# jperezrua/mfas

Hardware: AMD Instinct MI355X
Metric: candidate-archs trained/sec (NTU inner loop) (higher is better)
Workload: dtype f32

## Files before the change

include/mfas_hip.h:

```cpp
#ifndef MFAS_HIP_H
#define MFAS_HIP_H

#include <stdint.h>

#ifdef __cplusplus
extern "C" {
#endif

#define MFAS_OK 0
#define MFAS_EINVAL -1
#define MFAS_EHIP -2
#define MFAS_ENOMEM -3

#define MFAS_MAX_CELLS 4
#define MFAS_MAX_TAPS 8

#define MFAS_DT_F32 0
#define MFAS_DT_BF16 1
#define MFAS_DT_F16 2

typedef struct mfas_hyper {
    int32_t R;
    int32_t C;
    int32_t B;
// ... 74 lines not shown
int mfas_population_forward(mfas_population* pop, int32_t k, const mfas_table* tab, int64_t row0,
                            int64_t nrows, float* logits, int64_t* corrects);

int mfas_population_forward_train(mfas_population* pop, int32_t k, const mfas_table* tab, int64_t row0, int32_t nrows,
                                  int32_t step_index, float* logits);

int mfas_population_backward(mfas_population* pop, int32_t k, const mfas_table* table, int64_t row0, int32_t nrows,
                             int32_t step_index, const float* dlogits);

int mfas_population_sweep_profile(const mfas_population* pop, int64_t* launches, double* total_ms,
                                  double* bytes_per_launch);
int mfas_population_set_profiling(mfas_population* pop, int32_t on);

int mfas_population_schedule(const mfas_population* pop, int32_t info[8]);

int mfas_population_plan(const mfas_hyper* hp, const int32_t* confs, const int32_t* n_cells, int32_t K, int32_t device,
                         int32_t chunk_cols, int32_t info[8]);

int mfas_stream_probe(int64_t bytes_per_plane, int32_t iters, double* gb_per_s);

int mfas_global_pool(const void* x, int32_t dtype, int64_t rows, int64_t inner, void* out, int32_t out_dtype,
                     void* hip_stream);

int mfas_range_push(const char* name);
int mfas_range_pop(void);

int mfas_tuning_describe(char* buf, int32_t cap);

int mfas_population_set_best_threshold(mfas_population* pop, double threshold);

// ... 7 lines not shown
```

mfas_amd/_lib.py:

```python
import ctypes as C
import os

_HERE = os.path.dirname(os.path.abspath(__file__))
LIB_PATH = os.environ.get("MFAS_LIB") or os.path.join(_HERE, "csrc", "libmfas_hip.so")

MFAS_DT = {"float32": 0, "bfloat16": 1, "float16": 2}
MAX_TAPS = 8


class mfas_hyper(C.Structure):
    _fields_ = [("R", C.c_int32), ("C", C.c_int32), ("B", C.c_int32), ("bn", C.c_int32),
                ("alphas", C.c_int32), ("multitask", C.c_int32), ("drpt", C.c_double),
                ("wd", C.c_double), ("beta1", C.c_double), ("beta2", C.c_double),
                ("adam_eps", C.c_double), ("bn_eps", C.c_double), ("bn_momentum", C.c_double),
                ("s_sizes", C.c_int32 * MAX_TAPS), ("v_sizes", C.c_int32 * MAX_TAPS), ("loss_mode", C.c_int32),
                ("allow_plain_cell", C.c_int32), ("f1_threshold", C.c_double), ("tap_bits", C.c_int32), ("order_per_candidate", C.c_int32)]


class mfas_table(C.Structure):
    _fields_ = [("s", C.c_void_p * MAX_TAPS), ("v", C.c_void_p * MAX_TAPS), ("vlogit", C.c_void_p),
                ("slogit", C.c_void_p), ("label", C.c_void_p), ("multilabel", C.c_void_p), ("N", C.c_int64),
                ("dtype", C.c_int32), ("_pad", C.c_int32)]


# ... 23 lines not shown
    L.mfas_population_destroy.argtypes = [P]
    L.mfas_population_destroy.restype = None
    L.mfas_population_param_count.argtypes = [P, C.c_int32]
    L.mfas_population_param_count.restype = C.c_int64
    L.mfas_population_set_params.argtypes = [P, C.c_int32, P]
    L.mfas_population_get_params.argtypes = [P, C.c_int32, C.c_int32, P]
    L.mfas_population_init.argtypes = [P, P]
    L.mfas_population_train.argtypes = [P, C.POINTER(mfas_table), C.POINTER(mfas_table), P, P, C.c_int32,
                                        C.c_int64, C.c_int32, P, P]
    L.mfas_population_forward.argtypes = [P, C.c_int32, C.POINTER(mfas_table), C.c_int64, C.c_int64, P, P]
    L.mfas_population_forward_train.argtypes = [P, C.c_int32, C.POINTER(mfas_table), C.c_int64, C.c_int32, C.c_int32, P]
    L.mfas_population_backward.argtypes = [P, C.c_int32, C.POINTER(mfas_table), C.c_int64, C.c_int32, C.c_int32, P]
    L.mfas_population_sweep_profile.argtypes = [P, P, P, P]
    L.mfas_population_schedule.argtypes = [P, P]
    L.mfas_population_plan.argtypes = [C.POINTER(mfas_hyper), P, P, C.c_int32, C.c_int32, C.c_int32, P]
    L.mfas_population_set_profiling.argtypes = [P, C.c_int32]
    L.mfas_population_set_pos_weight.argtypes = [P, P]
    L.mfas_stream_probe.argtypes = [C.c_int64, C.c_int32, P]
    L.mfas_global_pool.argtypes = [P, C.c_int32, C.c_int64, C.c_int64, P, C.c_int32, P]
    L.mfas_range_push.argtypes = [C.c_char_p]
    L.mfas_population_init_torch_streams.argtypes = [P, P, P, C.c_double, C.c_double]
    L.mfas_tuning_describe.argtypes = [C.c_char_p, C.c_int32]
    L.mfas_population_train_from.argtypes = [P, C.POINTER(mfas_table), C.POINTER(mfas_table), P, P, C.c_int32,
                                             C.c_int32, C.c_int32, C.c_int32, P, P]
    L.mfas_population_set_state.argtypes = [P, C.c_int32, C.c_int32, P]
    L.mfas_population_get_progress.argtypes = [P, C.c_int32, P, P, P, P]
    L.mfas_population_set_progress.argtypes = [P, C.c_int32, P, P, P, P]
    L.mfas_population_move.argtypes = [P, C.c_int32, P, C.c_int32]
    _lib = L
    return L


EXPORTS = ["mfas_last_error", "mfas_version", "mfas_population_create", "mfas_population_destroy",
           "mfas_population_param_count", "mfas_population_set_params", "mfas_population_get_params",
           "mfas_population_init", "mfas_population_train", "mfas_population_forward",
           "mfas_population_sweep_profile", "mfas_population_set_profiling", "mfas_population_set_pos_weight", "mfas_global_pool", "mfas_stream_probe", "mfas_source_digest",
           "mfas_population_set_best_threshold", "mfas_population_forward_train", "mfas_population_schedule",
           "mfas_population_plan", "mfas_population_backward", "mfas_range_push", "mfas_range_pop", "mfas_population_init_torch_streams", "mfas_tuning_describe",
           "mfas_population_train_from", "mfas_population_set_state", "mfas_population_get_progress", "mfas_population_set_progress",
           "mfas_population_move"]


def tuning() -> dict:
    buf = C.create_string_buffer(2048)
    check(lib().mfas_tuning_describe(buf, 2048))
    return dict(kv.split("=", 1) for kv in buf.value.decode().split())


import contextlib


@contextlib.contextmanager
def profiler_range(name: str):
    L = lib()
    L.mfas_range_push(name.encode())
# ... 10 lines not shown
```

mfas_amd/csrc/launches.hip.h:

```cpp
#pragma once
#include <stdint.h>
#include <vector>

struct Launch {
    int sweep_g = -1, upd = 0, fwd = 0;
    int64_t sweep_t = 0;
    int chain_g = -1;
    int64_t chain_t = 0;
    int gather_g = -1, gather_n = 0;
    int64_t gather_b = 0;
};

static void epoch_launches(int ngroups, bool same_group, int64_t T, bool gather, std::vector<Launch>& out) {
    out.clear();
    gather = gather && ngroups == 2;
    auto add = [&](int gs, int upd, int fwd, int64_t ts, int gc, int64_t tc) -> Launch& {
        out.push_back(Launch{gs, upd, fwd, ts, gc, tc});
        return out.back();
    };
    auto rows = [&](Launch& l, int g, int64_t b, int n) { if (gather) { l.gather_g = g; l.gather_b = b; l.gather_n = n; } };
    for (int g = 0; g < ngroups; ++g) rows(add(g, 0, 1, 0, -1, 0), g, 0, T > 1 ? 2 : 1);
    if (ngroups == 1 && same_group) {
        for (int64_t t = 0; t < T; ++t) add(0, 1, t + 1 < T, t, 0, t);
    } else if (ngroups == 1) {
        for (int64_t t = 0; t < T; ++t) { add(-1, 0, 0, 0, 0, t); add(0, 1, t + 1 < T, t, -1, 0); }
    } else {
        add(-1, 0, 0, 0, 0, 0);
        for (int64_t t = 0; t < T; ++t) {
            const int fwd = t + 1 < T;
            Launch& a = add(0, 1, fwd, t, 1, t);
            if (t >= 1 && t + 1 < T) rows(a, 1, t + 1, 1);
            Launch& b = add(1, 1, fwd, t, fwd ? 0 : -1, t + 1);
            if (fwd && t + 2 < T) rows(b, 0, t + 2, 1);
        }
    }
}
```

mfas_amd/csrc/mfas_hip.hip:

```cpp
#include <hip/hip_runtime.h>
#include <hip/hip_fp16.h>
#pragma clang fp contract(off)
#include <stdint.h>
#include <stdio.h>
#include <string.h>
#include <math.h>
#include <algorithm>
#include <string>
#include <vector>
#include <thread>
#include <chrono>
#include <dlfcn.h>

#include "mfas_hip.h"

#include "common.hip.h"
#include "sweep.hip.h"
#include "chain.hip.h"

struct StepArgs {
    SweepArgs sa;
    ChainArgs ca;
    int32_t nchain, _pad;
    GatherArgs ga;
// ... 36 lines not shown
}

#include "wide.hip.h"
#include "persist.hip.h"
#include "eval.hip.h"
#include "pack.hip.h"

#include "plan.hip.h"

struct mfas_population {
    mfas_hyper hp;
    Tuning tune;
    int K = 0, device = 0, n_cus = 0;
    int chunk_cols_req = 0;
    hipStream_t stream = nullptr;
    LayoutPlan plan;
    float* plane = nullptr;
    float* wt = nullptr;
    float* stepbuf = nullptr;
    float* best = nullptr;
    CandDev* d_cands = nullptr;
    SegDesc* d_descs = nullptr;
    struct GroupDev { SegDesc* d_descs = nullptr; TapDesc* d_taps = nullptr; };
    std::vector<GroupDev> groups;
    DevStats* d_stats = nullptr;
    int32_t* d_status = nullptr;
    uint32_t* d_seeds = nullptr;
    long long* d_corr = nullptr;
    float* d_posw = nullptr;
    int stats_cap = 0;
// ... 188 lines not shown
    CREATE_CHK(hipMalloc(&p->d_corr, sizeof(long long)));
    CREATE_CHK(upload(&p->d_posw, std::vector<float>(pl.g.Cp, 1.0f)));
    CREATE_CHK(upload(&p->d_cands, pl.cands));
    CREATE_CHK(upload(&p->d_descs, pl.descs));
    p->groups.resize(pl.groups.size());
    for (size_t gi = 0; gi < pl.groups.size(); ++gi) {
        CREATE_CHK(upload(&p->groups[gi].d_descs, pl.groups[gi].descs));
        CREATE_CHK(upload(&p->groups[gi].d_taps, pl.groups[gi].taps));
    }
    if (pl.red_in_sweep) {
        CREATE_CHK(hipMalloc(&p->d_red_cnt, sizeof(uint32_t) * K * MFAS_MAX_CELLS));
        CREATE_CHK(hipMemset(p->d_red_cnt, 0, sizeof(uint32_t) * K * MFAS_MAX_CELLS));
    }
    if (pl.same_group) CREATE_CHK(hipMalloc(&p->d_cellflag, sizeof(uint32_t) * K * CELLFLAG_STRIDE));
    if (pl.chain_split) CREATE_CHK(hipMalloc(&p->d_xch, sizeof(float) * (size_t)K * XCH_CAND_FLOATS));
    CREATE_CHK(hipMemsetAsync(p->plane, 0, sizeof(float) * 3 * (size_t)pl.plane_stride, p->stream));
    CREATE_CHK(hipMemsetAsync(p->wt, 0, sizeof(float) * wt_floats, p->stream));
    CREATE_CHK(hipMemsetAsync(p->stepbuf, 0, sizeof(float) * (size_t)pl.step_total, p->stream));
    CREATE_CHK(set_lds_all(pl));
    if (pl.persist) {
        CREATE_CHK(upload(&p->d_pdescs, pl.pdescs));
        CREATE_CHK(upload(&p->d_need, pl.need));
        CREATE_CHK(upload(&p->d_role, pl.role));
        CREATE_CHK(hipMalloc(&p->d_sync, sizeof(uint32_t) * ((size_t)K * PERSIST_SYNC_STRIDE + 64)));
        if (p->tune.persist_trace) {
            CREATE_CHK(hipMalloc(&p->d_trace, sizeof(unsigned long long) * 256));
            CREATE_CHK(hipMemset(p->d_trace, 0, sizeof(unsigned long long) * 256));
        }
    }
    CREATE_CHK(hipStreamSynchronize(p->stream));
// ... 12 lines not shown
                                    int32_t chunk_cols, int32_t info[8]) {
    if (!info) return fail(MFAS_EINVAL, "null argument or K <= 0");
    if (int vrc = validate_inputs(hp, confs, n_cells, K)) return vrc;
    const int ncu = device_cus(device);
    LayoutPlan pl;
    if (int prc = plan_layout(hp, confs, n_cells, nullptr, K, chunk_cols, ncu, true, tuning_from_env(), pl)) return prc;
    info[0] = pl.persist ? 1 : 0; info[1] = pl.nres; info[2] = pl.nres_wg; info[3] = pl.res_nu;
    info[4] = pl.chunk; info[5] = (pl.lean_chain ? 1 : 0) | (pl.wide ? 2 : 0); info[6] = ncu; info[7] = K;
    return MFAS_OK;
}

extern "C" void mfas_population_destroy(mfas_population* p) {
    if (!p) return;
    hipSetDevice(p->device);
    hipStreamSynchronize(p->stream);
    for (hipEvent_t e : p->ev) hipEventDestroy(e);
    hipFree(p->plane); hipFree(p->wt); hipFree(p->stepbuf); hipFree(p->best);
    for (auto& gr : p->groups) { hipFree(gr.d_descs); hipFree(gr.d_taps); }
    hipFree(p->d_cands); hipFree(p->d_descs); hipFree(p->d_stats); hipFree(p->d_status);
    hipFree(p->d_seeds); hipFree(p->d_corr); hipFree(p->d_posw);
    hipFree(p->d_red_cnt);
    hipFree(p->d_gather);
    hipFree(p->d_cellflag);
    hipFree(p->d_xch);
    hipFree(p->d_move);
    hipFree(p->d_sync); hipFree(p->d_need); hipFree(p->d_role); hipFree(p->d_scal); hipFree(p->d_trace); hipFree(p->d_pdescs);
    delete p;
}

extern "C" int64_t mfas_population_param_count(const mfas_population* p, int32_t k) {
// ... 214 lines not shown
}

extern "C" int mfas_population_set_best_threshold(mfas_population* p, double threshold) {
    if (!p) return fail(MFAS_EINVAL, "null");
    p->best_threshold = threshold;
    return MFAS_OK;
}

extern "C" int mfas_population_set_profiling(mfas_population* p, int32_t on) {
    if (!p) return fail(MFAS_EINVAL, "null");
    p->profiling = on != 0;
    p->prof_every = p->tune.prof_every;
    return MFAS_OK;
}

extern "C" int mfas_population_schedule(const mfas_population* p, int32_t info[8]) {
    if (!p || !info) return fail(MFAS_EINVAL, "null");
    const LayoutPlan& pl = p->plan;
    info[0] = pl.persist ? 1 : 0; info[1] = pl.nres; info[2] = pl.nres_wg; info[3] = pl.res_nu;
    info[4] = pl.res_chain ? 1 : 0; info[5] = (pl.lean_chain ? 1 : 0) | (pl.wide ? 2 : 0) | (std::max(1, pl.chain_split) << 8); info[6] = pl.same_group ? -1 : (int32_t)pl.groups.size(); info[7] = p->K;
    return MFAS_OK;
}

extern "C" int mfas_population_sweep_profile(const mfas_population* p, int64_t* launches, double* total_ms,
                                             double* bytes_per_launch) {
    if (!p) return fail(MFAS_EINVAL, "null");
    if (launches) *launches = p->prof_launches;
    if (total_ms) *total_ms = p->prof_ms;
    if (bytes_per_launch) *bytes_per_launch = p->bytes_per_launch;
    return MFAS_OK;
}
```

mfas_amd/csrc/plan.hip.h:

```cpp
#pragma once
struct Tuning {
    int persist = -1;
    int no_lean_chain = 0;
    int groups = 0;
    int same_group = -1;
    int no_tap_major = 0;
    int force_tap_major = 0;
    int no_red_in_sweep = 0;
    double occ_bytes = -1.0;
    int no_xcd_placement = 0;
    int n_xcd = 0;
    int persist_trace = 0;
    int nt = -1;
    int eval_no_x16 = 0;
    int eval_no_msplit = 0;
    int eval_no_b3 = 0;
    int eval_no_wl = 0;
    int no_gather = 0;
    int gather_verbose = 0;
    int no_plain_chain = 0;
    int persist_verbose = 0;
    int prof_every = 16;
    int chain_split = -1;
    int test_not_resident = -1;
    int test_lose_step = -1;
};

static Tuning tuning_from_env() {
    Tuning t;
    auto flag = [](const char* n) { return getenv(n) ? 1 : 0; };
    auto num = [](const char* n, int dflt) { const char* e = getenv(n); return e ? atoi(e) : dflt; };
    t.persist = getenv("MFAS_PERSIST") ? (atoi(getenv("MFAS_PERSIST")) != 0 ? 1 : 0) : -1;
    t.no_lean_chain = flag("MFAS_NO_LEAN_CHAIN");
    t.groups = num("MFAS_GROUPS", 0);
    t.same_group = num("MFAS_SAME_GROUP", -1);
    t.no_tap_major = flag("MFAS_NO_TAP_MAJOR");
    t.force_tap_major = flag("MFAS_FORCE_TAP_MAJOR");
    t.no_red_in_sweep = flag("MFAS_NO_RED_IN_SWEEP");
    if (const char* e = getenv("MFAS_OCC_BYTES")) t.occ_bytes = atof(e);
    t.no_xcd_placement = flag("MFAS_NO_XCD_PLACEMENT");
    t.n_xcd = num("MFAS_XCDS", 0);
    t.persist_trace = flag("MFAS_PERSIST_TRACE");
    t.nt = getenv("MFAS_NT") ? (atoi(getenv("MFAS_NT")) != 0 ? 1 : 0) : -1;
    t.eval_no_x16 = flag("MFAS_EVAL_NO_X16");
    t.eval_no_msplit = flag("MFAS_EVAL_NO_MSPLIT");
    t.eval_no_b3 = flag("MFAS_EVAL_NO_B3");
    t.eval_no_wl = flag("MFAS_EVAL_NO_WL");
    t.no_gather = flag("MFAS_NO_GATHER");
    t.gather_verbose = flag("MFAS_GATHER_VERBOSE");
    t.no_plain_chain = flag("MFAS_NO_PLAIN_CHAIN");
    t.persist_verbose = num("MFAS_PERSIST_VERBOSE", 0);
    t.prof_every = std::max(1, num("MFAS_PROF_EVERY", 16));
    t.chain_split = num("MFAS_CHAIN_SPLIT", -1);
#ifdef MFAS_TEST_HOOKS
    t.test_not_resident = num("MFAS_PERSIST_TEST_NOT_RESIDENT", -1);
    t.test_lose_step = num("MFAS_PERSIST_TEST_LOSE_STEP", -1);
#endif
    return t;
}

extern "C" int mfas_tuning_describe(char* buf, int32_t cap) {
    if (!buf || cap <= 0) return MFAS_EINVAL;
    const Tuning t = tuning_from_env();
    char tmp[1024];
    snprintf(tmp, sizeof(tmp),
             "persist=%d no_lean_chain=%d groups=%d same_group=%d "
             "no_tap_major=%d force_tap_major=%d no_red_in_sweep=%d occ_bytes=%g no_xcd_placement=%d n_xcd=%d persist_trace=%d nt=%d eval_no_x16=%d "
             "eval_no_msplit=%d eval_no_b3=%d eval_no_wl=%d no_gather=%d gather_verbose=%d no_plain_chain=%d persist_verbose=%d prof_every=%d "
             "chain_split=%d test_not_resident=%d test_lose_step=%d hooks=%d",
             t.persist, t.no_lean_chain, t.groups, t.same_group,
             t.no_tap_major, t.force_tap_major, t.no_red_in_sweep, t.occ_bytes, t.no_xcd_placement, t.n_xcd, t.persist_trace, t.nt, t.eval_no_x16,
             t.eval_no_msplit, t.eval_no_b3, t.eval_no_wl, t.no_gather, t.gather_verbose, t.no_plain_chain, t.persist_verbose, t.prof_every,
             t.chain_split, t.test_not_resident, t.test_lose_step,
#ifdef MFAS_TEST_HOOKS
             1
#else
             0
#endif
    );
    snprintf(buf, (size_t)cap, "%s", tmp);
    return MFAS_OK;
}

static inline int ceil16(int x) { return (x + 15) & ~15; }

static int pick_chunk(int cols_p, int target) {
    int best = 16;
    for (int c = 16; c <= cols_p && c <= target; c += 16)
        if (cols_p % c == 0) best = c;
    return best;
}

static int validate_inputs(const mfas_hyper* hp, const int32_t* confs, const int32_t* n_cells, int32_t K) {
    if (!hp || !confs || !n_cells || K <= 0) return fail(MFAS_EINVAL, "null argument or K <= 0");
// ... 156 lines not shown
    std::vector<int64_t> nparams;
    std::vector<int64_t> cand_plane_base, cand_plane_size;
    int64_t plane_stride = 0, wt_size = 0, step_total = 0;
    double bytes_per_launch = 0.0;
    bool persist = false;
    bool res_chain = false;
    bool res_wide = false;
    int nres = 0;
    int res_nu = 1;
    int nres_wg = 0;
    int res_buf_words = 0;
    bool wide = false;
    std::vector<int> wide_start;
    bool lean_chain = false;
    bool same_group = false;
    int chain_split = 0;
    bool red_in_sweep = false;
    bool nontemporal = false;
    double occ_bytes = 0;
    int mbe = 4, nrbw = 1;
    bool yf_in_lds = false, vec_in_lds = false;
    size_t lds_step = 0, lds_chain = 0, lds_eval = 0;
    bool fits_lds = false;
    size_t lds_split = 0;
    size_t lds_president = 0;
    std::vector<GroupPlan> groups;
    std::vector<SegDesc> pdescs;
    std::vector<int32_t> need;
    std::vector<int32_t> role;
};
// ... 166 lines not shown
        if (pl.lds_eval <= 80 * 1024) break;
    }
    pl.fits_lds = !(pl.mbe < 1 || pl.nrbw > 8 || pl.lds_step > 150 * 1024 || (wide && pl.lds_chain > 150 * 1024));

    {
        int ngroups = pl.lean_chain ? ((K >= 40 && K < 224) ? 2 : 1) : (K >= 8 ? 2 : 1);
        if (tu.groups > 0) ngroups = (tu.groups >= 2 && K >= 2) ? 2 : 1;
        if (pl.persist || wide) ngroups = 1;
        {
            const int sgenv = tu.same_group;
            double state_bytes = 0;
            for (const SegDesc& d : pl.descs) state_bytes += 24.0 * d.cc * d.rows_p;
            const bool two_forced = tu.groups >= 2;
            pl.same_group = !wide && !pl.persist && !pl.lean_chain && g.MB <= 2 && (state_bytes <= 260e6 || sgenv == 2) && sgenv != 0 && !two_forced;
        }
        if (pl.same_group) ngroups = 1;
        pl.chain_split = ((pl.same_group || (ngroups == 2 && K < 28)) && !pl.lean_chain && !pl.persist && g.MB == 1 && g.nrb == 8 && g.ncb <= 4 && !g.alphas &&
                          tu.chain_split != 0 && tu.chain_split != 1) ? 4 : 0;
        int split = K;
        if (ngroups == 2) {
            double tot = 0, run = 0;
            for (const SegDesc& d : pl.descs) tot += (double)d.cc * d.rows_p;
            split = 1;
            for (int k = 0; k < K - 1; ++k) {
                for (int j = pl.desc_start[k]; j < pl.desc_start[k + 1]; ++j) run += (double)pl.descs[j].cc * pl.descs[j].rows_p;
                split = k + 1;
                if (run >= tot / 2) break;
            }
        }
        for (int gi = 0; gi < ngroups; ++gi) {
            pl.groups.emplace_back();
            GroupPlan& gr = pl.groups.back();
            gr.c0 = gi == 0 ? 0 : split;
            gr.nc = gi == 0 ? split : K - split;
            std::vector<SegDesc> all(pl.descs.begin() + pl.desc_start[gr.c0], pl.descs.begin() + pl.desc_start[gr.c0 + gr.nc]);
            for (const SegDesc& d : all) {
                gr.alg_state += 24.0 * d.rows * std::max(0, std::min(d.cc, d.cols - d.k0));
                if (d.kind <= KIND_V) gr.alg_feat += (double)hp->B * d.cc;
            }
            std::vector<SegDesc>& sorted = gr.descs;
            std::vector<TapDesc>& taps = gr.taps;
            const bool tap_major = !wide && (g.nrb == 1 || g.nrb == 2 || g.nrb == 4) && !tu.no_tap_major && !pl.persist && !pl.same_group &&
                                   !hp->order_per_candidate;
            if (tap_major) {
// ... 141 lines not shown
```

mfas_amd/csrc/train.hip.h:

```cpp
#pragma once
struct TrainCall {
    mfas_population* p = nullptr;
    const mfas_table *train = nullptr, *dev = nullptr;
    const int32_t* order = nullptr; const float* step_scalars = nullptr;
    int epochs = 0, first = 0, last = 0, B = 0;
    bool segment = false, resume = false, do_dev = false, snapshot_best = false;
    int64_t max_steps = -1, N = 0, nb = 0;
    AdamC ac; StepArgs st;
    std::vector<Launch> launches;
    int64_t launches_T = -1;
    int64_t split_launches[2] = {0, 0};
    size_t ev_used = 0;
    std::vector<double> ev_bytes; int64_t nlaunch = 0;
    bool use_gather = false;
    int64_t g_par_stride = 0, g_cand_stride = 0;
    std::vector<uint32_t> aborts;
    std::vector<double> best_acc;
    double metric_scale = 1.0; std::vector<DevStats> hstats;
    int elt() const { return train->dtype == MFAS_DT_F32 ? 4 : 2; }
    double dev_metric(int k, int ep) const { return (double)hstats[(size_t)k * epochs + ep].dev_corr * metric_scale / (double)dev->N; }
};

static void base_args(mfas_population* p, const mfas_table& tab, const int32_t* order, const Geo& g, const AdamC& ac, SweepArgs& sa, ChainArgs& ca) {
    const LayoutPlan& pl = p->plan;
    sa.cands = p->d_cands; sa.plane = p->plane; sa.plane_stride = pl.plane_stride; sa.wt = p->wt;
    sa.stepbuf = p->stepbuf; sa.tab = tab; sa.order = order; sa.g = g; sa.ac = ac;
    ca.plane = p->plane; ca.plane_stride = pl.plane_stride; ca.wt = p->wt; ca.stepbuf = p->stepbuf;
    ca.tab = tab; ca.order = order; ca.g = g; ca.status = p->d_status; ca.ac = ac;
    ca.yf_in_lds = pl.yf_in_lds ? 1 : 0; ca.vec_in_lds = pl.vec_in_lds ? 1 : 0; ca.pos_w = p->d_posw;
}

static hipError_t setup_gather(TrainCall& c) {
    mfas_population* p = c.p;
    const Geo& g = c.st.sa.g;
    c.use_gather = p->plan.groups.size() == 2 && !p->plan.persist && c.order && g.order_stride > 0 && !p->tune.no_gather;
    if (!c.use_gather) return hipSuccess;
    int64_t totw = 0;
    for (int u = 0; u < MFAS_MAX_TAPS; ++u) totw += g.sw[u] + g.vw[u];
    c.g_par_stride = totw * g.Bp * c.elt(); c.g_cand_stride = 2 * c.g_par_stride;
    const size_t need = (size_t)c.g_cand_stride * p->K;
    if (p->gather_cap < need) {
        hipFree(p->d_gather); p->d_gather = nullptr; p->gather_cap = 0;
        hipError_t e = hipMalloc(&p->d_gather, need);
        if (e != hipSuccess) { c.use_gather = false; (void)hipGetLastError(); return hipSuccess; }
        p->gather_cap = need;
    }
    if (p->tune.gather_verbose) fprintf(stderr, "[gather] on: %d candidates, %.1f MB of gathered rows\n", p->K, (double)need / 1e6);
    return hipSuccess;
}

// ... 11 lines not shown
    if (pl.red_in_sweep) e_ = hipMemsetAsync(p->d_red_cnt, 0, sizeof(uint32_t) * K * MFAS_MAX_CELLS, p->stream);
    if (e_ == hipSuccess && pl.same_group) e_ = hipMemsetAsync(p->d_cellflag, 0, sizeof(uint32_t) * K * CELLFLAG_STRIDE, p->stream);
    if (e_ == hipSuccess && pl.chain_split) e_ = hipMemsetAsync(p->d_xch, 0xFF, sizeof(float) * (size_t)K * XCH_CAND_FLOATS, p->stream);
    st.ca.xch = p->d_xch; st.ca.nsplit = pl.chain_split; st.ca.xpar = 0;
    c.split_launches[0] = c.split_launches[1] = 0;
    if (e_ == hipSuccess && ep > 0 && pl.same_group && pl.chain_split)
        e_ = hipMemsetD32Async(reinterpret_cast<hipDeviceptr_t>(p->d_cellflag), (int)((uint32_t)pl.chain_split * (uint32_t)(ep * c.nb)),
                               (size_t)K * CELLFLAG_STRIDE, p->stream);
    return e_ != hipSuccess ? e_ : setup_gather(c);
}

struct ProfBracket {
    TrainCall& c;
    const bool on;
    const double bytes;
    ProfBracket(TrainCall& c_, bool on_, double bytes_) : c(c_), on(on_), bytes(bytes_) {
        if (!on) return;
        mfas_population* p = c.p;
        if (p->ev.size() < c.ev_used + 2) {
            hipEvent_t e0, e1;
            hipEventCreate(&e0); hipEventCreate(&e1); p->ev.push_back(e0); p->ev.push_back(e1);
        }
        hipEventRecord(p->ev[c.ev_used], p->stream);
    }
    ~ProfBracket() {
        if (!on) return;
        hipEventRecord(c.p->ev[c.ev_used + 1], c.p->stream);
        c.ev_used += 2; c.ev_bytes.push_back(bytes);
    }
};

static StepKernel pick_step_kernel(const LayoutPlan& pl, const Launch& L, unsigned nch, bool same, bool split) {
    const int MB = pl.g.MB;
    if (pl.wide) return wide_sweep_kernel(pl.nontemporal);
    if (same) return same_kernel(MB, pl.nontemporal, split ? pl.chain_split : 1);
    if (split) return step_kernel(MB, pl.nontemporal, 4, false, pl.chain_split);
    const bool occ = nch == 0 || pl.groups[L.sweep_g].alg_state > pl.occ_bytes;
    return step_kernel(MB, pl.nontemporal, MB == 1 || (MB == 2 && (occ || pl.lean_chain)) ? 4 : 2, pl.lean_chain, 1);
}

static void launch_record(TrainCall& c, int64_t ep, const Launch& L) {
    mfas_population* p = c.p;
    const LayoutPlan& pl = p->plan;
    StepArgs& st = c.st;
    const int64_t N = c.N;
    const int B = c.B, gs = L.sweep_g, gc = L.chain_g;
    auto nvalid = [&](int64_t t) { return (int)std::min<int64_t>(B, N - t * B); };
    unsigned nsw = 0, nch = 0;
    st.ga.nblocks = 0; st.ga.nsets = 0; st.sa.gather = nullptr;
    if (c.use_gather) {
        GatherArgs& ga = st.ga;
        ga.buf = p->d_gather; ga.cand_stride = c.g_cand_stride; ga.par_stride = c.g_par_stride;
        for (int s = 0; s < L.gather_n; ++s) {
            const int64_t t = L.gather_b + s;
            ga.pos[s] = ep * N + t * B; ga.base[s] = (int)(t * B); ga.nvalid[s] = nvalid(t); ga.par[s] = (int)(t & 1);
        }
        if (L.gather_g >= 0) { ga.nsets = L.gather_n; ga.cands = p->d_cands + pl.groups[L.gather_g].c0; ga.nblocks = pl.groups[L.gather_g].nc; }
        if (gs >= 0 && L.upd) {
            st.sa.gather = p->d_gather; st.sa.g_cand_stride = c.g_cand_stride; st.sa.g_par_stride = c.g_par_stride;
            st.sa.g_par_t = (int)(L.sweep_t & 1); st.sa.g_par_n = (int)((L.sweep_t + 1) & 1);
        }
// ... 9 lines not shown
        s.ac.ss = L.upd ? c.step_scalars[2 * gstep] : 0.f;
        s.ac.bc2s = L.upd ? c.step_scalars[2 * gstep + 1] : 1.f;
        nsw = (unsigned)(pl.groups[gs].descs.size() + pl.groups[gs].taps.size());
    } else st.sa.ntap = 0;
    if (gc >= 0) {
        ChainArgs& ca = st.ca;
        const int64_t tc = L.chain_t, gstep = ep * c.nb + tc;
        ca.cands = p->d_cands + pl.groups[gc].c0;
        ca.pos_t = ep * N + tc * B; ca.base_t = (int)(tc * B); ca.nvalid = nvalid(tc);
        ca.gstep = (int)gstep; ca.epoch = (int)ep;
        ca.ac.ss = c.step_scalars[2 * gstep]; ca.ac.bc2s = c.step_scalars[2 * gstep + 1];
        nch = (unsigned)pl.groups[gc].nc;
    }
    st.nchain = (int)nch;
    if (nsw == 0) {
        launch(pl.wide ? wide_chain_kernel() : chain_kernel(pl.g.MB, pl.lean_chain), nch, pl.lds_chain, p->stream, st.ca);
        return;
    }
    ProfBracket prof(c, p->profiling && L.upd && L.fwd && ((c.nlaunch++ % p->prof_every) == 0),
                     pl.groups[gs].alg_state + pl.groups[gs].alg_feat * c.elt() + 8.0 * B * pl.groups[gs].nc);
    const bool same = pl.same_group && gc == gs && L.upd, split = pl.chain_split && nch > 0;
    if (split) {
        st.ca.ncand = (int)nch; st.ca.xpar = (int)(c.split_launches[gc & 1]++ & 1);
        st.nchain = pl.chain_split * (int)((nch + 7) & ~7u);
    }
    if (same) {
        st.sa.cellflag = p->d_cellflag; st.ca.cellflag = p->d_cellflag;
        st.sa.flag_target = st.ca.flag_target = (split ? (uint32_t)pl.chain_split : 1u) * ((uint32_t)st.ca.gstep + 1u);
        st.sa.flag_status = p->d_status;
    }
    launch(pick_step_kernel(pl, L, nch, same, split), (unsigned)st.nchain + st.ga.nblocks + nsw, split ? pl.lds_split : pl.lds_step, p->stream, st);
    if (same) { st.sa.cellflag = nullptr; st.ca.cellflag = nullptr; }
}

static hipError_t persist_epoch_once(TrainCall& c, int ep, int64_t T) {
    mfas_population* p = c.p;
    const LayoutPlan& pl = p->plan;
    const Geo& g = pl.g;
    const int K = p->K;
    if (p->tune.test_not_resident >= 0 && ep >= p->tune.test_not_resident) { c.aborts[ep] = PERSIST_ABORT_NOT_RESIDENT; return hipSuccess; }
    hipError_t e = hipMemsetAsync(p->d_sync, 0, sizeof(uint32_t) * ((size_t)K * PERSIST_SYNC_STRIDE + 64), p->stream);
    if (e != hipSuccess) return e;
    PersistArgs pa;
    memset(&pa, 0, sizeof(pa));
    pa.sa = c.st.sa; pa.ca = c.st.ca;
    pa.sa.desc = p->d_pdescs; pa.sa.tdesc = nullptr; pa.sa.ntap = 0;
    pa.ca.cands = p->d_cands;
    pa.nchain = K; pa.nitems = (int)pl.pdescs.size(); pa.nres = pl.nres; pa.res_chain = pl.res_chain ? 1 : 0; pa.res_wide = pl.res_wide ? 1 : 0;
    pa.res_nu = pl.res_nu; pa.nres_wg = pl.nres_wg; pa.res_buf_words = pl.res_buf_words;
    pa.T = (int)T; pa.epoch = ep;
    pa.lose_step = p->tune.test_lose_step;
    pa.N = c.N; pa.pos0 = (int64_t)ep * c.N;
    pa.B = c.B; pa.gstep0 = (int)((int64_t)ep * c.nb);
    pa.scal = p->d_scal; pa.sync = p->d_sync; pa.need = p->d_need; pa.role = p->d_role; pa.trace = p->d_trace;
    const unsigned grid = (unsigned)(K + pa.nres_wg);
    if ((int)grid > p->n_cus) return hipErrorInvalidConfiguration;
    {
        ProfBracket prof(c, p->profiling, (double)T * (pl.groups[0].alg_state + pl.groups[0].alg_feat * c.elt() + 8.0 * c.B * K));
        const int lw = (int)(pl.lds_president / 4) - PERSIST_LDS_WORDS;
        const bool simple = !g.alphas && !g.multitask && g.loss_mode == 0 && !p->tune.no_plain_chain;
        const bool x16 = c.train->dtype != MFAS_DT_F32;
        launch(president_kernel(g.MB, x16, x16 && pl.res_wide, pl.res_nu, simple ? (g.bn ? 2 : 1) : 0), grid, pl.lds_president, p->stream, pa, lw);
    }
    e = hipGetLastError();
    if (e != hipSuccess) return e;
    return hipMemcpyAsync(&c.aborts[ep], p->d_sync + (size_t)K * PERSIST_SYNC_STRIDE, sizeof(uint32_t), hipMemcpyDeviceToHost, p->stream);
}

static hipError_t persist_epoch(TrainCall& c, int ep, int64_t T) {
    mfas_population* p = c.p;
    for (int attempt = 0;; ++attempt) {
        hipError_t e = persist_epoch_once(c, ep, T);
        if (e != hipSuccess) return e;
// ... 118 lines not shown
    HIPCHK(init_args(c, c.first));
    p->prof_launches = 0; p->prof_ms = 0.0; p->prof_bytes = 0.0;
    if (p->plan.persist) {
        const int64_t steps = (int64_t)epochs * c.nb;
        if (p->scal_cap < (size_t)steps * 2) {
            hipFree(p->d_scal); p->d_scal = nullptr;
            HIPCHK(hipMalloc(&p->d_scal, sizeof(float) * steps * 2));
            p->scal_cap = (size_t)steps * 2;
        }
        const size_t have = (size_t)(c.max_steps >= 0 ? std::min<int64_t>(c.max_steps, steps) : steps) * 2;
        HIPCHK(hipMemcpyAsync(p->d_scal, c.step_scalars, sizeof(float) * have, hipMemcpyHostToDevice, p->stream));
    }
    return MFAS_OK;
}

static int train_epoch(TrainCall& c, int ep, int64_t T) {
    mfas_population* p = c.p;
    if (p->plan.persist) {
        HIPCHK(persist_epoch(c, ep, T));
        if (c.aborts[ep] == PERSIST_ABORT_NOT_RESIDENT) {
            if (p->tune.persist_verbose) fprintf(stderr, "[persist] epoch %d: the resident grid never became resident; falling back to launch-per-phase\n", ep);
            if (int rc = persist_fallback(p)) return rc;
            HIPCHK(init_args(c, ep));
            c.aborts[ep] = 0;
        } else if (c.aborts[ep]) {
            HIPCHK(hipStreamSynchronize(p->stream));
            return fail(MFAS_EHIP, "persistent step loop: a workgroup timed out waiting for its dependency (abort code 1: the epoch was "
                                   "abandoned half way, this population's parameters are not usable)");
        }
    }
    if (!p->plan.persist) {
        if (c.launches_T != T) { epoch_launches((int)p->plan.groups.size(), p->plan.same_group, T, c.use_gather, c.launches); c.launches_T = T; }
        for (const Launch& L : c.launches) launch_record(c, ep, L);
    }
    HIPCHK(hipGetLastError());
    return MFAS_OK;
}

static int train_dev(TrainCall& c, int ep) {
    mfas_population* p = c.p;
    const int K = p->K;
    EvalArgs ea;
    memset(&ea, 0, sizeof(ea));
    ea.cands = p->d_cands; ea.plane = p->plane; ea.tab = *c.dev; ea.row0 = 0; ea.nrows = c.dev->N;
    ea.cand0 = 0; ea.epoch = ep; ea.E = c.epochs; ea.g = c.st.sa.g; ea.stats = p->d_stats; ea.pos_w = p->d_posw;
    HIPCHK(launch_eval(p, ea, K, p->stream));
    if (!c.snapshot_best) return MFAS_OK;
    HIPCHK(hipMemcpyAsync(c.hstats.data(), p->d_stats, sizeof(DevStats) * K * c.epochs, hipMemcpyDeviceToHost, p->stream));
// ... 51 lines not shown
        p->bytes_per_launch = p->prof_launches ? p->prof_bytes / p->prof_launches : 0.0;
    }
    return MFAS_OK;
}

static int train_impl(mfas_population* p, const mfas_table* train, const mfas_table* dev, const int32_t* order, const float* step_scalars,
                      int32_t epochs, int64_t max_steps, int32_t snapshot_best, mfas_epoch_stats* stats, int32_t* status,
                      const int32_t first, const int32_t last, const bool segment) {
    TrainCall c;
    c.p = p; c.train = train; c.dev = dev; c.order = order; c.step_scalars = step_scalars; c.epochs = epochs; c.max_steps = max_steps;
    c.snapshot_best = snapshot_best != 0; c.first = first; c.last = last; c.segment = segment;
    if (int rc = train_check(c, stats)) return rc;
    RangeGuard call_range("mfas_population_train K=" + std::to_string(p->K) + " R=" + std::to_string(p->plan.g.R) + " B=" + std::to_string(c.B) +
                          " E=" + std::to_string(epochs) + (p->plan.persist ? " resident" : " launch-per-phase"));
    if (int rc = train_begin(c)) return rc;
    int64_t done = 0;
    for (int ep = first; ep < last; ++ep) {
        const int64_t T = max_steps >= 0 ? std::min<int64_t>(c.nb, max_steps - done) : c.nb;
        if (T <= 0) break;
        RangeGuard epoch_range("epoch " + std::to_string(ep));
        if (int rc = train_epoch(c, ep, T)) return rc;
        done += T;
        if (c.do_dev) if (int rc = train_dev(c, ep)) return rc;
    }
    return train_end(c, stats, status);
}

static int single_batch(mfas_population* p, int32_t k, const mfas_table* tab, int64_t row0, int32_t nrows, int32_t step_index,
                        float* logits, const float* dlogits) {
    if (!p || (!logits && !dlogits) || k < 0 || k >= p->K || row0 < 0) return fail(MFAS_EINVAL, "bad argument");
    if (int rc = check_table(p, tab, false)) return rc;
    const LayoutPlan& pl = p->plan;
    if (nrows < 1 || nrows > pl.g.B) return fail(MFAS_EINVAL, "train-mode forward: 1 <= rows <= the population's batch size");
    if (nrows == 1 && pl.g.bn) return fail(MFAS_EINVAL, "train-mode BatchNorm needs more than 1 row (reference: ValueError)");
    if (row0 + nrows > tab->N) return fail(MFAS_EINVAL, "row range outside the table");
    HIPCHK(hipSetDevice(p->device));
// ... 37 lines not shown
```

mfas_amd/engine.py:

```python
from __future__ import annotations

import ctypes as C
import math
from dataclasses import dataclass
from typing import Dict, List, Optional, Sequence

import numpy as np
import torch

from . import _lib
from .scheduler import adam_step_scalars

S_SIZES = (128, 256, 1024, 512)
V_SIZES = (512, 1024, 2048, 2048)
TAPS = tuple(f"s{j}" for j in range(_lib.MAX_TAPS)) + tuple(f"v{j}" for j in range(_lib.MAX_TAPS))


@dataclass
class Hyper:
    R: int = 16
    C: int = 60
    B: int = 20
    bn: bool = False
    drpt: float = 0.5
# ... 428 lines not shown

    def set_pos_weight(self, w):
        w = np.ascontiguousarray(np.asarray(w, np.float32))
        assert w.size == self.hp.C
        _lib.check(self.lib.mfas_population_set_pos_weight(self._h, w.ctypes.data))

    def set_best_threshold(self, threshold: float):
        _lib.check(self.lib.mfas_population_set_best_threshold(self._h, float(threshold)))

    def set_profiling(self, on: bool):
        _lib.check(self.lib.mfas_population_set_profiling(self._h, int(on)))

    def schedule(self):
        info = (C.c_int32 * 8)()
        _lib.check(self.lib.mfas_population_schedule(self._h, info))
        keys = ("persistent", "resident_units", "resident_workgroups", "units_per_workgroup", "resident_chain", "lean_chain", "groups", "candidates")
        d = dict(zip(keys, (int(x) for x in info)))
        d["chain_cus"] = max(1, (d["lean_chain"] >> 8) & 0xFF)
        d["wide"] = (d["lean_chain"] >> 1) & 1
        d["lean_chain"] &= 1
        return d

    def sweep_profile(self):
        n, ms, by = C.c_int64(0), C.c_double(0), C.c_double(0)
        _lib.check(self.lib.mfas_population_sweep_profile(self._h, C.byref(n), C.byref(ms), C.byref(by)))
        return int(n.value), float(ms.value), float(by.value)


def save_checkpoint(path: str, pop: Population):
    import dataclasses
    cands = []
    for k in range(pop.K):
        st = pop.export_candidate(k)
        cands.append({key: (v.cpu() if torch.is_tensor(v) else v) for key, v in st.items()})
    hyper = {key: (list(v) if isinstance(v, (tuple, list)) else v) for key, v in dataclasses.asdict(pop.hp).items()}
    torch.save({"format": 1, "hyper": hyper, "confs": [c.tolist() for c in pop.confs], "candidates": cands}, path)


def load_checkpoint(path: str, pop: Population):
    import dataclasses
    ck = torch.load(path, map_location="cpu", weights_only=True)
# ... 19 lines not shown
    for k, c in enumerate(confs):
        if not 1 <= len(c) <= 4:
            raise ValueError("a configuration has 1..4 fusion cells")
        cf[k, :len(c)] = c
        nc[k] = len(c)
    dev = torch.device(device)
    idx = dev.index if dev.index is not None else torch.cuda.current_device()
    info = np.zeros(8, np.int32)
    hc = hp.to_c()
    _lib.check(lib.mfas_population_plan(C.byref(hc), cf.ctypes.data, nc.ctypes.data, len(confs), int(idx), int(chunk_cols), info.ctypes.data))
    return {"persistent": bool(info[0]), "resident_units": int(info[1]), "resident_workgroups": int(info[2]),
            "units_per_workgroup": int(info[3]), "chunk_cols": int(info[4]), "lean_chain": bool(info[5] & 1), "wide": bool(info[5] & 2), "compute_units": int(info[6]),
            "candidates": int(info[7])}


def best_dev_f1(stats_row, status_nan: bool, n_dev: int, init_f1: float = 0.0):
    best = init_f1
    for e in range(len(stats_row)):
        if status_nan and not np.isfinite(stats_row["train_loss_sum"][e]):
            break
        f1 = float(stats_row["dev_corrects"][e]) / F1_FIXED_POINT / float(n_dev)
        if f1 > best:
            best = f1
    return 0.0 if best != best else best


def best_dev_accuracy(stats_row, n_dev: int) -> float:
    best = 0.0
    for e in range(len(stats_row)):
        acc = float(stats_row["dev_corrects"][e]) / float(n_dev)
# ... 4 lines not shown
```

Baseline: 34.44.

## Add optional two-stream schedule splitting candidate groups across HIP streams

Adds an opt-in mode (MFAS_STREAMS=2) that splits candidates into two halves. Each half gets its own same-group launch sequence on a separate non-blocking stream, joined with fork/join events. The aim is to let the two halves' step kernels overlap on the GPU instead of serialising on one stream. It also gates chain splitting on whether the chain workgroups fit in the available CUs, which can change the default schedule for large populations. A plan_schedule query API is added for inspection.

```diff
diff --git a/include/mfas_hip.h b/include/mfas_hip.h
--- a/include/mfas_hip.h
+++ b/include/mfas_hip.h
@@ -112,6 +112,9 @@
 
 int mfas_population_schedule(const mfas_population* pop, int32_t info[8]);
 
+int mfas_population_plan_schedule(const mfas_hyper* hp, const int32_t* confs, const int32_t* n_cells, int32_t K, int32_t n_cus,
+                                  int32_t chunk_cols, int32_t info[8]);
+
 int mfas_population_plan(const mfas_hyper* hp, const int32_t* confs, const int32_t* n_cells, int32_t K, int32_t device,
                          int32_t chunk_cols, int32_t info[8]);
 
diff --git a/mfas_amd/_lib.py b/mfas_amd/_lib.py
--- a/mfas_amd/_lib.py
+++ b/mfas_amd/_lib.py
@@ -61,6 +61,7 @@
     L.mfas_population_sweep_profile.argtypes = [P, P, P, P]
     L.mfas_population_schedule.argtypes = [P, P]
     L.mfas_population_plan.argtypes = [C.POINTER(mfas_hyper), P, P, C.c_int32, C.c_int32, C.c_int32, P]
+    L.mfas_population_plan_schedule.argtypes = [C.POINTER(mfas_hyper), P, P, C.c_int32, C.c_int32, C.c_int32, P]
     L.mfas_population_set_profiling.argtypes = [P, C.c_int32]
     L.mfas_population_set_pos_weight.argtypes = [P, P]
     L.mfas_stream_probe.argtypes = [C.c_int64, C.c_int32, P]
@@ -85,7 +86,7 @@
            "mfas_population_set_best_threshold", "mfas_population_forward_train", "mfas_population_schedule",
            "mfas_population_plan", "mfas_population_backward", "mfas_range_push", "mfas_range_pop", "mfas_population_init_torch_streams", "mfas_tuning_describe",
            "mfas_population_train_from", "mfas_population_set_state", "mfas_population_get_progress", "mfas_population_set_progress",
-           "mfas_population_move"]
+           "mfas_population_move", "mfas_population_plan_schedule"]
 
 
 def tuning() -> dict:
diff --git a/mfas_amd/csrc/launches.hip.h b/mfas_amd/csrc/launches.hip.h
--- a/mfas_amd/csrc/launches.hip.h
+++ b/mfas_amd/csrc/launches.hip.h
@@ -9,18 +9,23 @@
     int64_t chain_t = 0;
     int gather_g = -1, gather_n = 0;
     int64_t gather_b = 0;
+    int stream = 0;
 };
 
 static void epoch_launches(int ngroups, bool same_group, int64_t T, bool gather, std::vector<Launch>& out) {
     out.clear();
-    gather = gather && ngroups == 2;
+    gather = gather && ngroups == 2 && !same_group;
     auto add = [&](int gs, int upd, int fwd, int64_t ts, int gc, int64_t tc) -> Launch& {
         out.push_back(Launch{gs, upd, fwd, ts, gc, tc});
         return out.back();
     };
     auto rows = [&](Launch& l, int g, int64_t b, int n) { if (gather) { l.gather_g = g; l.gather_b = b; l.gather_n = n; } };
     for (int g = 0; g < ngroups; ++g) rows(add(g, 0, 1, 0, -1, 0), g, 0, T > 1 ? 2 : 1);
-    if (ngroups == 1 && same_group) {
+    if (ngroups == 2 && same_group) {
+        for (int64_t t = 0; t < T; ++t)
+            for (int g = 0; g < 2; ++g) add(g, 1, t + 1 < T, t, g, t);
+        for (Launch& l : out) l.stream = l.sweep_g;
+    } else if (ngroups == 1 && same_group) {
         for (int64_t t = 0; t < T; ++t) add(0, 1, t + 1 < T, t, 0, t);
     } else if (ngroups == 1) {
         for (int64_t t = 0; t < T; ++t) { add(-1, 0, 0, 0, 0, t); add(0, 1, t + 1 < T, t, -1, 0); }
diff --git a/mfas_amd/csrc/mfas_hip.hip b/mfas_amd/csrc/mfas_hip.hip
--- a/mfas_amd/csrc/mfas_hip.hip
+++ b/mfas_amd/csrc/mfas_hip.hip
@@ -74,6 +74,8 @@
     int K = 0, device = 0, n_cus = 0;
     int chunk_cols_req = 0;
     hipStream_t stream = nullptr;
+    hipStream_t stream2 = nullptr;
+    hipEvent_t ev_fork = nullptr, ev_join = nullptr;
     LayoutPlan plan;
     float* plane = nullptr;
     float* wt = nullptr;
@@ -292,6 +294,11 @@
     }
     if (pl.same_group) CREATE_CHK(hipMalloc(&p->d_cellflag, sizeof(uint32_t) * K * CELLFLAG_STRIDE));
     if (pl.chain_split) CREATE_CHK(hipMalloc(&p->d_xch, sizeof(float) * (size_t)K * XCH_CAND_FLOATS));
+    if (pl.two_stream) {
+        CREATE_CHK(hipStreamCreateWithFlags(&p->stream2, hipStreamNonBlocking));
+        CREATE_CHK(hipEventCreateWithFlags(&p->ev_fork, hipEventDisableTiming));
+        CREATE_CHK(hipEventCreateWithFlags(&p->ev_join, hipEventDisableTiming));
+    }
     CREATE_CHK(hipMemsetAsync(p->plane, 0, sizeof(float) * 3 * (size_t)pl.plane_stride, p->stream));
     CREATE_CHK(hipMemsetAsync(p->wt, 0, sizeof(float) * wt_floats, p->stream));
     CREATE_CHK(hipMemsetAsync(p->stepbuf, 0, sizeof(float) * (size_t)pl.step_total, p->stream));
@@ -334,6 +341,9 @@
     if (!p) return;
     hipSetDevice(p->device);
     hipStreamSynchronize(p->stream);
+    if (p->stream2) { hipStreamSynchronize(p->stream2); hipStreamDestroy(p->stream2); }
+    if (p->ev_fork) hipEventDestroy(p->ev_fork);
+    if (p->ev_join) hipEventDestroy(p->ev_join);
     for (hipEvent_t e : p->ev) hipEventDestroy(e);
     hipFree(p->plane); hipFree(p->wt); hipFree(p->stepbuf); hipFree(p->best);
     for (auto& gr : p->groups) { hipFree(gr.d_descs); hipFree(gr.d_taps); }
@@ -578,11 +588,25 @@
     return MFAS_OK;
 }
 
+static void schedule_info(const LayoutPlan& pl, int K, int32_t info[8]) {
+    info[0] = pl.persist ? 1 : 0; info[1] = pl.nres; info[2] = pl.nres_wg; info[3] = pl.res_nu;
+    info[4] = pl.res_chain ? 1 : 0; info[5] = (pl.lean_chain ? 1 : 0) | (pl.wide ? 2 : 0) | (pl.two_stream ? 4 : 0) | (std::max(1, pl.chain_split) << 8);
+    info[6] = pl.same_group && !pl.two_stream ? -1 : (int32_t)pl.groups.size(); info[7] = K;
+}
+
 extern "C" int mfas_population_schedule(const mfas_population* p, int32_t info[8]) {
     if (!p || !info) return fail(MFAS_EINVAL, "null");
-    const LayoutPlan& pl = p->plan;
-    info[0] = pl.persist ? 1 : 0; info[1] = pl.nres; info[2] = pl.nres_wg; info[3] = pl.res_nu;
-    info[4] = pl.res_chain ? 1 : 0; info[5] = (pl.lean_chain ? 1 : 0) | (pl.wide ? 2 : 0) | (std::max(1, pl.chain_split) << 8); info[6] = pl.same_group ? -1 : (int32_t)pl.groups.size(); info[7] = p->K;
+    schedule_info(p->plan, p->K, info);
+    return MFAS_OK;
+}
+
+extern "C" int mfas_population_plan_schedule(const mfas_hyper* hp, const int32_t* confs, const int32_t* n_cells, int32_t K, int32_t n_cus,
+                                             int32_t chunk_cols, int32_t info[8]) {
+    if (!info || n_cus <= 0) return fail(MFAS_EINVAL, "null argument or n_cus <= 0");
+    if (int vrc = validate_inputs(hp, confs, n_cells, K)) return vrc;
+    LayoutPlan pl;
+    if (int prc = plan_layout(hp, confs, n_cells, nullptr, K, chunk_cols, n_cus, true, tuning_from_env(), pl)) return prc;
+    schedule_info(pl, K, info);
     return MFAS_OK;
 }
 
diff --git a/mfas_amd/csrc/plan.hip.h b/mfas_amd/csrc/plan.hip.h
--- a/mfas_amd/csrc/plan.hip.h
+++ b/mfas_amd/csrc/plan.hip.h
@@ -22,6 +22,7 @@
     int persist_verbose = 0;
     int prof_every = 16;
     int chain_split = -1;
+    int streams = -1;
     int test_not_resident = -1;
     int test_lose_step = -1;
 };
@@ -52,6 +53,8 @@
     t.persist_verbose = num("MFAS_PERSIST_VERBOSE", 0);
     t.prof_every = std::max(1, num("MFAS_PROF_EVERY", 16));
     t.chain_split = num("MFAS_CHAIN_SPLIT", -1);
+    t.streams = num("MFAS_STREAMS", -1);
+    if (t.streams != 1 && t.streams != 2) t.streams = -1;
 #ifdef MFAS_TEST_HOOKS
     t.test_not_resident = num("MFAS_PERSIST_TEST_NOT_RESIDENT", -1);
     t.test_lose_step = num("MFAS_PERSIST_TEST_LOSE_STEP", -1);
@@ -78,6 +81,7 @@
              0
 #endif
     );
+    if (t.streams != -1) snprintf(tmp + strlen(tmp), sizeof(tmp) - strlen(tmp), " streams=%d", t.streams);
     snprintf(buf, (size_t)cap, "%s", tmp);
     return MFAS_OK;
 }
@@ -264,6 +268,7 @@
     std::vector<int> wide_start;
     bool lean_chain = false;
     bool same_group = false;
+    bool two_stream = false;
     int chain_split = 0;
     bool red_in_sweep = false;
     bool nontemporal = false;
@@ -460,20 +465,27 @@
             const bool two_forced = tu.groups >= 2;
             pl.same_group = !wide && !pl.persist && !pl.lean_chain && g.MB <= 2 && (state_bytes <= 260e6 || sgenv == 2) && sgenv != 0 && !two_forced;
         }
-        if (pl.same_group) ngroups = 1;
-        pl.chain_split = ((pl.same_group || (ngroups == 2 && K < 28)) && !pl.lean_chain && !pl.persist && g.MB == 1 && g.nrb == 8 && g.ncb <= 4 && !g.alphas &&
-                          tu.chain_split != 0 && tu.chain_split != 1) ? 4 : 0;
-        int split = K;
-        if (ngroups == 2) {
+        int half = K;
+        if (K >= 2) {
             double tot = 0, run = 0;
             for (const SegDesc& d : pl.descs) tot += (double)d.cc * d.rows_p;
-            split = 1;
+            half = 1;
             for (int k = 0; k < K - 1; ++k) {
                 for (int j = pl.desc_start[k]; j < pl.desc_start[k + 1]; ++j) run += (double)pl.descs[j].cc * pl.descs[j].rows_p;
-                split = k + 1;
+                half = k + 1;
                 if (run >= tot / 2) break;
             }
         }
+        pl.two_stream = tu.streams == 2 && !wide && !pl.persist && !pl.lean_chain && g.MB <= 2 && K >= 2;
+        if (pl.two_stream) { pl.same_group = true; ngroups = 2; }
+        else if (pl.same_group) ngroups = 1;
+        {
+            auto ceil8 = [](int x) { return (x + 7) & ~7; };
+            const int chain_wgs = pl.two_stream ? 4 * (ceil8(half) + ceil8(K - half)) : ngroups == 2 ? 4 * ceil8(std::max(half, K - half)) : 4 * ceil8(K);
+            pl.chain_split = ((pl.same_group || (ngroups == 2 && K < 28)) && !pl.lean_chain && !pl.persist && g.MB == 1 && g.nrb == 8 && g.ncb <= 4 && !g.alphas &&
+                              tu.chain_split != 0 && tu.chain_split != 1 && chain_wgs <= n_cus) ? 4 : 0;
+        }
+        const int split = ngroups == 2 ? half : K;
         for (int gi = 0; gi < ngroups; ++gi) {
             pl.groups.emplace_back();
             GroupPlan& gr = pl.groups.back();
diff --git a/mfas_amd/csrc/train.hip.h b/mfas_amd/csrc/train.hip.h
--- a/mfas_amd/csrc/train.hip.h
+++ b/mfas_amd/csrc/train.hip.h
@@ -11,7 +11,8 @@
     int64_t launches_T = -1;
     int64_t split_launches[2] = {0, 0};
     size_t ev_used = 0;
-    std::vector<double> ev_bytes; int64_t nlaunch = 0;
+    std::vector<double> ev_bytes; int64_t nlaunch[2] = {0, 0};
+    bool forked = false;
     bool use_gather = false;
     int64_t g_par_stride = 0, g_cand_stride = 0;
     std::vector<uint32_t> aborts;
@@ -33,7 +34,7 @@
 static hipError_t setup_gather(TrainCall& c) {
     mfas_population* p = c.p;
     const Geo& g = c.st.sa.g;
-    c.use_gather = p->plan.groups.size() == 2 && !p->plan.persist && c.order && g.order_stride > 0 && !p->tune.no_gather;
+    c.use_gather = p->plan.groups.size() == 2 && !p->plan.two_stream && !p->plan.persist && c.order && g.order_stride > 0 && !p->tune.no_gather;
     if (!c.use_gather) return hipSuccess;
     int64_t totw = 0;
     for (int u = 0; u < MFAS_MAX_TAPS; ++u) totw += g.sw[u] + g.vw[u];
@@ -75,18 +76,19 @@
     TrainCall& c;
     const bool on;
     const double bytes;
-    ProfBracket(TrainCall& c_, bool on_, double bytes_) : c(c_), on(on_), bytes(bytes_) {
+    hipStream_t stream;
+    ProfBracket(TrainCall& c_, bool on_, double bytes_, hipStream_t stream_) : c(c_), on(on_), bytes(bytes_), stream(stream_) {
         if (!on) return;
         mfas_population* p = c.p;
         if (p->ev.size() < c.ev_used + 2) {
             hipEvent_t e0, e1;
             hipEventCreate(&e0); hipEventCreate(&e1); p->ev.push_back(e0); p->ev.push_back(e1);
         }
-        hipEventRecord(p->ev[c.ev_used], p->stream);
+        hipEventRecord(p->ev[c.ev_used], stream);
     }
     ~ProfBracket() {
         if (!on) return;
-        hipEventRecord(c.p->ev[c.ev_used + 1], c.p->stream);
+        hipEventRecord(c.p->ev[c.ev_used + 1], stream);
         c.ev_used += 2; c.ev_bytes.push_back(bytes);
     }
 };
@@ -106,6 +108,7 @@
     StepArgs& st = c.st;
     const int64_t N = c.N;
     const int B = c.B, gs = L.sweep_g, gc = L.chain_g;
+    const hipStream_t stream = L.stream ? p->stream2 : p->stream;
     auto nvalid = [&](int64_t t) { return (int)std::min<int64_t>(B, N - t * B); };
     unsigned nsw = 0, nch = 0;
     st.ga.nblocks = 0; st.ga.nsets = 0; st.sa.gather = nullptr;
@@ -145,11 +148,11 @@
     }
     st.nchain = (int)nch;
     if (nsw == 0) {
-        launch(pl.wide ? wide_chain_kernel() : chain_kernel(pl.g.MB, pl.lean_chain), nch, pl.lds_chain, p->stream, st.ca);
+        launch(pl.wide ? wide_chain_kernel() : chain_kernel(pl.g.MB, pl.lean_chain), nch, pl.lds_chain, stream, st.ca);
         return;
     }
-    ProfBracket prof(c, p->profiling && L.upd && L.fwd && ((c.nlaunch++ % p->prof_every) == 0),
-                     pl.groups[gs].alg_state + pl.groups[gs].alg_feat * c.elt() + 8.0 * B * pl.groups[gs].nc);
+    ProfBracket prof(c, p->profiling && L.upd && L.fwd && ((c.nlaunch[gs & 1]++ % p->prof_every) == 0),
+                     pl.groups[gs].alg_state + pl.groups[gs].alg_feat * c.elt() + 8.0 * B * pl.groups[gs].nc, stream);
     const bool same = pl.same_group && gc == gs && L.upd, split = pl.chain_split && nch > 0;
     if (split) {
         st.ca.ncand = (int)nch; st.ca.xpar = (int)(c.split_launches[gc & 1]++ & 1);
@@ -160,7 +163,7 @@
         st.sa.flag_target = st.ca.flag_target = (split ? (uint32_t)pl.chain_split : 1u) * ((uint32_t)st.ca.gstep + 1u);
         st.sa.flag_status = p->d_status;
     }
-    launch(pick_step_kernel(pl, L, nch, same, split), (unsigned)st.nchain + st.ga.nblocks + nsw, split ? pl.lds_split : pl.lds_step, p->stream, st);
+    launch(pick_step_kernel(pl, L, nch, same, split), (unsigned)st.nchain + st.ga.nblocks + nsw, split ? pl.lds_split : pl.lds_step, stream, st);
     if (same) { st.sa.cellflag = nullptr; st.ca.cellflag = nullptr; }
 }
 
@@ -187,7 +190,7 @@
     const unsigned grid = (unsigned)(K + pa.nres_wg);
     if ((int)grid > p->n_cus) return hipErrorInvalidConfiguration;
     {
-        ProfBracket prof(c, p->profiling, (double)T * (pl.groups[0].alg_state + pl.groups[0].alg_feat * c.elt() + 8.0 * c.B * K));
+        ProfBracket prof(c, p->profiling, (double)T * (pl.groups[0].alg_state + pl.groups[0].alg_feat * c.elt() + 8.0 * c.B * K), p->stream);
         const int lw = (int)(pl.lds_president / 4) - PERSIST_LDS_WORDS;
         const bool simple = !g.alphas && !g.multitask && g.loss_mode == 0 && !p->tune.no_plain_chain;
         const bool x16 = c.train->dtype != MFAS_DT_F32;
@@ -336,6 +339,16 @@
     return MFAS_OK;
 }
 
+static hipError_t join_streams(TrainCall& c) {
+    mfas_population* p = c.p;
+    if (!c.forked) return hipSuccess;
+    c.forked = false;
+    hipError_t e = hipEventRecord(p->ev_join, p->stream2);
+    if (e == hipSuccess) e = hipStreamWaitEvent(p->stream, p->ev_join, 0);
+    if (e != hipSuccess) { (void)hipStreamSynchronize(p->stream2); (void)hipStreamSynchronize(p->stream); }
+    return e;
+}
+
 static int train_epoch(TrainCall& c, int ep, int64_t T) {
     mfas_population* p = c.p;
     if (p->plan.persist) {
@@ -352,8 +365,16 @@
         }
     }
     if (!p->plan.persist) {
-        if (c.launches_T != T) { epoch_launches((int)p->plan.groups.size(), p->plan.same_group, T, c.use_gather, c.launches); c.launches_T = T; }
-        for (const Launch& L : c.launches) launch_record(c, ep, L);
+        const bool two = p->plan.two_stream;
+        if (c.launches_T != T) {
+            epoch_launches((int)p->plan.groups.size(), p->plan.same_group, T, c.use_gather, c.launches);
+            c.launches_T = T;
+        }
+        for (const Launch& L : c.launches) {
+            if (two && L.stream && !c.forked) { HIPCHK(hipEventRecord(p->ev_fork, p->stream)); c.forked = true; HIPCHK(hipStreamWaitEvent(p->stream2, p->ev_fork, 0)); }
+            launch_record(c, ep, L);
+        }
+        if (two) HIPCHK(join_streams(c));
     }
     HIPCHK(hipGetLastError());
     return MFAS_OK;
@@ -435,12 +456,13 @@
     RangeGuard call_range("mfas_population_train K=" + std::to_string(p->K) + " R=" + std::to_string(p->plan.g.R) + " B=" + std::to_string(c.B) +
                           " E=" + std::to_string(epochs) + (p->plan.persist ? " resident" : " launch-per-phase"));
     if (int rc = train_begin(c)) return rc;
+    auto failed = [&c](int rc) { if (c.forked) { (void)join_streams(c); (void)hipStreamSynchronize(c.p->stream); } return rc; };
     int64_t done = 0;
     for (int ep = first; ep < last; ++ep) {
         const int64_t T = max_steps >= 0 ? std::min<int64_t>(c.nb, max_steps - done) : c.nb;
         if (T <= 0) break;
         RangeGuard epoch_range("epoch " + std::to_string(ep));
-        if (int rc = train_epoch(c, ep, T)) return rc;
+        if (int rc = train_epoch(c, ep, T)) return failed(rc);
         done += T;
         if (c.do_dev) if (int rc = train_dev(c, ep)) return rc;
     }
diff --git a/mfas_amd/engine.py b/mfas_amd/engine.py
--- a/mfas_amd/engine.py
+++ b/mfas_amd/engine.py
@@ -466,17 +466,23 @@
     def schedule(self):
         info = (C.c_int32 * 8)()
         _lib.check(self.lib.mfas_population_schedule(self._h, info))
-        keys = ("persistent", "resident_units", "resident_workgroups", "units_per_workgroup", "resident_chain", "lean_chain", "groups", "candidates")
-        d = dict(zip(keys, (int(x) for x in info)))
-        d["chain_cus"] = max(1, (d["lean_chain"] >> 8) & 0xFF)
-        d["wide"] = (d["lean_chain"] >> 1) & 1
-        d["lean_chain"] &= 1
-        return d
+        return _schedule_dict(info)
 
     def sweep_profile(self):
         n, ms, by = C.c_int64(0), C.c_double(0), C.c_double(0)
         _lib.check(self.lib.mfas_population_sweep_profile(self._h, C.byref(n), C.byref(ms), C.byref(by)))
         return int(n.value), float(ms.value), float(by.value)
+
+
+def _schedule_dict(info) -> Dict[str, int]:
+    keys = ("persistent", "resident_units", "resident_workgroups", "units_per_workgroup", "resident_chain", "lean_chain", "groups", "candidates")
+    d = dict(zip(keys, (int(x) for x in info)))
+    d["chain_cus"] = max(1, (d["lean_chain"] >> 8) & 0xFF)
+    d["wide"] = (d["lean_chain"] >> 1) & 1
+    if (d["lean_chain"] >> 2) & 1:
+        d["streams"] = 2
+    d["lean_chain"] &= 1
+    return d
 
 
 def save_checkpoint(path: str, pop: Population):
@@ -526,6 +532,20 @@
             "candidates": int(info[7])}
 
 
+def plan_schedule(hp: Hyper, confs: Sequence[np.ndarray], n_cus: int = 256, chunk_cols: int = 0) -> Dict[str, int]:
+    confs = [np.asarray(c, dtype=np.int64).reshape(-1, 3) for c in confs]
+    cf = np.zeros((len(confs), 4, 3), np.int32)
+    nc = np.zeros(len(confs), np.int32)
+    for k, c in enumerate(confs):
+        cf[k, :len(c)] = c
+        nc[k] = len(c)
+    info = np.zeros(8, np.int32)
+    hc = hp.to_c()
+    _lib.check(_lib.lib().mfas_population_plan_schedule(C.byref(hc), cf.ctypes.data, nc.ctypes.data, len(confs), int(n_cus), int(chunk_cols),
+                                                        info.ctypes.data))
+    return _schedule_dict(info)
+
+
 def best_dev_f1(stats_row, status_nan: bool, n_dev: int, init_f1: float = 0.0):
     best = init_f1
     for e in range(len(stats_row)):
```

New measurement: 33.81. 0.982x the previous value.
